# CVMethods/gabor_color_image_segmentation

Hardware: AMD Instinct MI355X
Metric: Mpix/s segmented (Gabor+k-means), 481x321x3 batch (higher is better)
Workload: dtype i8; 1 GPU; batch 64/GPU synthetic 481x321x3 uint8 (seed 0), 4-scale x 6-orientation Gabor bank ksize 13 on a 2-level octave pyramid, k=8, n_iter=10; codebook=global, global_batch=64, parallelism=dp1 (images sharded, int64 centroid all-reduce)

## Files before the change

### gabor_color_image_segmentation_amd/csrc/lloyd_mfma.hip

```cpp
#include "lloyd_pass.h"


#ifndef GCS_KP_WAVES
#define GCS_KP_WAVES 3
#endif
#ifndef GCS_ABL
#define GCS_ABL 0
#endif
#ifdef GCS_KP_PHASES
__device__ unsigned long long g_kp_phases[1024 * 4 * 8];
extern "C" int gcs_debug_kp_phases(unsigned long long *out) {
    return (int)hipMemcpyFromSymbol(out, HIP_SYMBOL(g_kp_phases), sizeof(unsigned long long) * 1024 * 4 * 8);
}
#define KP_PHASE_DECL unsigned long long kp_ph[6] = {0, 0, 0, 0, 0, 0}, kp_t0 = __builtin_amdgcn_s_memtime(), kp_tiles = 0
#define KP_PHASE(k)                                                   \
    do {                                                              \
        const unsigned long long t_ = __builtin_amdgcn_s_memtime();   \
        kp_ph[k] += t_ - kp_t0;                                       \
        kp_t0 = t_;                                                   \
    } while (0)
#define KP_PHASE_STORE                                                                                           \
    do {                                                                                                         \
        const int wg_ = (int)(blockIdx.y * gridDim.x + blockIdx.x);                                              \
        if (lane == 0 && wg_ < 1024) {                                                                           \
            for (int k_ = 0; k_ < 6; ++k_) g_kp_phases[(wg_ * 4 + (wid & 3)) * 8 + k_] = kp_ph[k_];             \
            g_kp_phases[(wg_ * 4 + (wid & 3)) * 8 + 6] = kp_tiles;                                               \
        }                                                                                                        \
    } while (0)
#else
#define KP_PHASE_DECL
#define KP_PHASE(k)
#define KP_PHASE_STORE
#endif

template <int KT, int NST, int DSTEPS, int WAVES, bool SPLIT = false, int L0T = 0, bool FUSED = false>
__global__ __launch_bounds__(64 * WAVES, (WAVES == 8 ? 2
                                          : DSTEPS == KP_DSTEPS_NARROW && KT == 1 && NST <= (SPLIT ? 3 : 6) ? GCS_KP_WAVES
                                          : DSTEPS == KP_DSTEPS_NARROW ? 2 : 1)) void kmeans_pass_mfma_kernel(
    const unsigned char *__restrict__ feats, const uint16_t *__restrict__ cent, GcsLayout lo, int K, int per_image,
    int parts, int reverse, int row_lo, int row_hi, uint64_t *__restrict__ partials, void *__restrict__ raster,
    int raster_u8, int nt_flag, GcsFold fz) {
    constexpr int KP_ROWS = 16 * DSTEPS, KP_DSTEPS = DSTEPS, KP_NT = 2 * DSTEPS;
    constexpr int NTHR = 64 * WAVES;
    constexpr int NT_OWN = WAVES == 8 ? (KP_NT + 1) / 2 : KP_NT;
    constexpr int KP_COARSE = DSTEPS == KP_DSTEPS_NARROW ? 40 * 32 + 64 : 104 * 32 + 64;
    __shared__ __attribute__((aligned(16))) unsigned char s_tile[KP_ROWS * KP_PITCH];
    __shared__ __attribute__((aligned(16))) unsigned char s_coarse[KP_COARSE];
    __shared__ __attribute__((aligned(16))) unsigned char s_lab[KP_TP];
    __shared__ long long s_const[16];
    constexpr int KP_FLAGS = 320;
    __shared__ unsigned char s_flag[SPLIT ? KP_FLAGS : 4];
    static_assert(!SPLIT || (DSTEPS == KP_DSTEPS_NARROW && WAVES == 4), "the split slab is the narrow pass's");
    static_assert(!FUSED || (SPLIT && KT == 1), "the self-updating pass exists for the CL1 kernels");

    const bool do_acc = partials != nullptr;
    const int tid = threadIdx.x, lane = tid & 63;
    const int wid = tid >> 6;
    const int wave = wid & 3;
    const int half = wid >> 2;
    const int b = blockIdx.y, part = blockIdx.x;
    const int D = lo.D;
    const uint16_t *cset = cent + (size_t)(per_image ? b : 0) * K * D;
    const int ntiles = lo.ntiles;
    const int nimg = per_image ? 1 : (int)gridDim.y;
    const int G = parts * nimg, g = per_image ? part : b * parts + part;
    const int nlist = ntiles * nimg;
    const unsigned char *fb = feats + (size_t)(per_image ? b : 0) * lo.img_bytes;

    uint16_t *cs = reinterpret_cast<uint16_t *>(s_tile);
    if constexpr (FUSED) {
        const int D1 = D + 1, row_len = K * D1;
        const int set = per_image ? b : 0;
        const int wg = b * (int)gridDim.x + part, nwg = (int)(gridDim.x * gridDim.y);
        {
            const long long total = (long long)(per_image ? (int)gridDim.y : 1) * fz.rows * row_len;
            for (long long i = (long long)wg * NTHR + tid; i < total; i += (long long)nwg * NTHR) fz.clear[i] = 0ull;
        }
        unsigned long long *fsum = reinterpret_cast<unsigned long long *>(s_tile + 8 * KT * KP_ROWS * 2);
        static_assert(8 * KT * KP_ROWS * 2 % 16 == 0 && 8 * KT * KP_ROWS * 2 + 8 * (8 * KT * KP_ROWS) <= KP_ROWS * KP_PITCH,
                      "the folded sums do not fit behind the centroid scratch");
        const bool later = fz.prev != nullptr;
        if (later) {
            const unsigned long long *pv = fz.prev + (size_t)set * fz.rows * row_len;
            for (int i = tid; i < row_len; i += NTHR) {
                unsigned long long s = 0;
                for (int r = 0; r < fz.rows; ++r) s += pv[(size_t)r * row_len + i];
                fsum[i] = s;
            }
            __syncthreads();
        }
        const bool writer = part == 0 && (per_image || b == 0);
        const long long P = (long long)lo.H * lo.W;
        for (int i = tid; i < 8 * KT * KP_ROWS; i += NTHR) {
            const int j = i / KP_ROWS, r = i % KP_ROWS;
            int e = 0;
            if (r >= lo.row0[0] && r < lo.row0[0] + lo.DL[0]) e = kp_logical_of<0>(lo, r - lo.row0[0]);
            if (lo.n_levels > 1 && r >= lo.row0[1] && r < lo.row0[1] + lo.DL[1]) e = kp_logical_of<1>(lo, r - lo.row0[1]);
            unsigned v = 0;
            if (j < K && r < D) {
                if (later) {
                    const unsigned long long c = fsum[j * D1 + D], s = fsum[j * D1 + e];
                    v = c > 0 ? (unsigned)((2 * s + c) / (2 * c)) : (unsigned)cset[j * D + e];
                } else {
                    const long long p = ((2LL * j + 1) * P) / (2LL * K);
                    v = gcs_slab_value(feats, lo, set, r, (int)(p / lo.W), (int)(p % lo.W));
                }
                if (writer) {
                    fz.cent_new[((size_t)set * K + j) * D + e] = (uint16_t)v;
                    fz.cent_out[((size_t)set * K + j) * D + e] = (uint16_t)v;
                }
                v ^= 0x8080u;
            }
            cs[i] = (uint16_t)v;
        }
    } else
    for (int i = tid; i < 8 * KT * KP_ROWS; i += NTHR) {
        const int j = i / KP_ROWS, r = i % KP_ROWS;
        int e = 0;
        if (r >= lo.row0[0] && r < lo.row0[0] + lo.DL[0]) e = kp_logical_of<0>(lo, r - lo.row0[0]);
        if (lo.n_levels > 1 && r >= lo.row0[1] && r < lo.row0[1] + lo.DL[1]) e = kp_logical_of<1>(lo, r - lo.row0[1]);
        if (lo.n_levels > 2 && r >= lo.row0[2] && r < lo.row0[2] + lo.DL[2]) e = kp_logical_of<2>(lo, r - lo.row0[2]);
        if (lo.n_levels > 3 && r >= lo.row0[3] && r < lo.row0[3] + lo.DL[3]) e = kp_logical_of<3>(lo, r - lo.row0[3]);
        cs[i] = (j < K && r < D) ? (uint16_t)(cset[j * D + e] ^ 0x8080u) : (uint16_t)0;
    }
    if constexpr (SPLIT) {
        for (int it = tid; it < KP_FLAGS; it += NTHR) {
            const long long lt = (long long)g + (long long)it * G;
            unsigned char f = 0;
            if (lt < nlist) {
                const int T = reverse ? nlist - 1 - (int)lt : (int)lt;
                const int bi = T / ntiles, tn = T - bi * ntiles;
                f = *reinterpret_cast<const unsigned *>(fb + (size_t)bi * lo.img_bytes + lo.flag_off + 4 * (size_t)tn) != 0u;
            }
            s_flag[it] = f;
        }
    }
    __syncthreads();
    {
      for (int j = tid >> 4; j < 16; j += NTHR / 16) {
        const int sub = tid & 15;
        long long nrm = 0, scl = 0, sch = 0;
        if (j < K)
            for (int d = sub; d < D; d += 16) {
                const long long c = cs[j * KP_ROWS + d] ^ 0x8080u;
                nrm += c * c;
                scl += c & 255;
                sch += c >> 8;
            }
#pragma unroll
        for (int m = 8; m >= 1; m >>= 1) {
            nrm += __shfl_xor(nrm, m);
            scl += __shfl_xor(scl, m);
            sch += __shfl_xor(sch, m);
        }
        if (sub == 0) {
            const long long q = 16384LL * D;
            const long long g = (128 * scl - q) + 256 * (128 * (sch + scl) - 2 * q) + 65536 * (128 * sch - q);
            s_const[j] = j < K ? 16 * (nrm - 2 * g) + j : (1LL << 62) + j;
        }
      }
    }
    v4i apat[KT][KP_DSTEPS];
    {
        const int r = lane & 31, h = lane >> 5;
        const int jj = r >> 2, pat = r & 3;
        const unsigned msk = pat == 0 ? 0x00ff00ffu : pat == 1 ? 0xffffffffu : pat == 2 ? 0xff00ff00u : 0u;
        const unsigned sel = pat == 1 ? 0x02030001u : 0x03020100u;
#pragma unroll
        for (int mt = 0; mt < KT; ++mt)
#pragma unroll
            for (int kk = 0; kk < KP_DSTEPS; ++kk) {
                const v4i w = *reinterpret_cast<const v4i *>(&cs[(8 * mt + jj) * KP_ROWS + 16 * kk + 8 * h]);
                v4i f;
#pragma unroll
                for (int e = 0; e < 4; ++e) f[e] = (int)(__builtin_amdgcn_perm(0u, (unsigned)w[e], sel) & msk);
                apat[mt][kk] = f;
            }
    }
    __syncthreads();
    constexpr bool CL1 = SPLIT && KT == 1;
    const int DL0 = lo.DL[0];
    auto row_addr = [&](int r) -> int {
        return CL1 && r >= DL0 ? DL0 * KP_PITCH + (r - DL0) * KP_P1 : r * KP_PITCH;
    };
    auto row_swz = [&](int r) -> int { return CL1 && r < DL0 ? ((r >> 3) & 1) * 32 : 0; };
    if (tid < (CL1 ? 32 : KP_TP / 2)) reinterpret_cast<unsigned *>(&s_tile[row_addr(D)])[tid] = 0x01010101u;
    constexpr bool UPD2 = SPLIT && KT == 1;
    constexpr int NACC = UPD2 ? DSTEPS : NT_OWN;
    v4i accu[NACC];
#pragma unroll
    for (int nt = 0; nt < NACC; ++nt) accu[nt] = v4i{0, 0, 0, 0};

    const int n0 = SPLIT ? 16 * lo.DL[0] : 32 * lo.DL[0];
    const int n1 = lo.n_levels > 1 ? 8 * lo.DL[1] : 0;
    const int nchunk = SPLIT ? lo.S >> 4 : lo.tile_bytes >> 4;
    v4i st[NST];
    v2i sm[NST], stt[NST];
#pragma unroll
    for (int i = 0; i < NST; ++i) stt[i] = v2i{0, 0};
    int sdst[NST], ssrc[NST];
    int scls[NST];
    bool sl1[NST];
#pragma unroll
    for (int i = 0; i < NST; ++i) {
        const int ci = min(tid + NTHR * i, nchunk - 1);
        ssrc[i] = ci;
        const int c1 = ci - n0;
        const bool l1 = SPLIT ? c1 >= 0 : c1 >= 0 && c1 < n1;
        sl1[i] = l1;
        if constexpr (SPLIT)
            sdst[i] = l1 ? (CL1 ? (int)(size_t)&s_tile[row_addr(lo.row0[1] + (c1 >> 2)) + (c1 & 3) * 32]
                                : (int)(size_t)&s_tile[(lo.row0[1] + (c1 >> 2)) * KP_PITCH + (c1 & 3) * 32])
                         : (int)(size_t)&s_tile[(ci >> 4) * KP_PITCH + (((ci & 1) * 256 + ((ci & 15) >> 1) * 16) ^ row_swz(ci >> 4))];
        else
            sdst[i] = ci < n0 ? (int)(size_t)&s_tile[(ci >> 5) * KP_PITCH + (ci & 31) * 16]
                      : l1    ? (int)(size_t)&s_tile[(lo.row0[1] + (c1 >> 3)) * KP_PITCH + (c1 & 7) * 64]
                              : (int)(size_t)&s_coarse[(c1 - n1) * 16];
        const unsigned long long m = __builtin_amdgcn_ballot_w64(l1);
        scls[i] = m == 0ull ? 0 : m == ~0ull ? 1 : 2;
    }
    auto stage_load = [&](int tile) {
        const v4i *src = reinterpret_cast<const v4i *>(fb + (size_t)tile * lo.tile_bytes);
#pragma unroll
        for (int i = 0; i < NST; ++i) st[i] = src[ssrc[i]];
    };
    auto stage_load_split = [&](const unsigned char *p_lo, unsigned mid_rel, bool top, bool nt) {
        const __amdgpu_buffer_rsrc_t rs = __builtin_amdgcn_make_buffer_rsrc(const_cast<unsigned char *>(p_lo), 0, -1, 0x00020000);
        const unsigned top_rel = mid_rel + (unsigned)(lo.top_off - lo.mid_off);
        auto go = [&](auto aux_c) {
            constexpr int AUX = decltype(aux_c)::value;
#pragma unroll
            for (int i = 0; i < NST; ++i) {
                const unsigned o = (unsigned)ssrc[i] * 16u;
                st[i] = __builtin_bit_cast(v4i, __builtin_amdgcn_raw_buffer_load_b128(rs, (int)o, 0, AUX));
                sm[i] = __builtin_bit_cast(v2i, __builtin_amdgcn_raw_buffer_load_b64(rs, (int)(o >> 1), (int)mid_rel, AUX));
            }
            if (top) {
#pragma unroll
                for (int i = 0; i < NST; ++i)
                    stt[i] = __builtin_bit_cast(v2i, __builtin_amdgcn_raw_buffer_load_b64(rs, (int)((unsigned)ssrc[i] * 8u), (int)top_rel, AUX));
            } else {
#pragma unroll
                for (int i = 0; i < NST; ++i) {
                    v2i u;
                    asm("" : "=v"(u));
                    stt[i] = u;
                }
            }
        };
        if (nt) go(std::integral_constant<int, 2>{});
        else go(std::integral_constant<int, 0>{});
    };
    typedef __attribute__((address_space(3))) v4i *lds_v4i_ptr;
    bool top_regs = false;
    auto stage_write_as = [&](auto topp) {
    constexpr bool TOPP = decltype(topp)::value;
    auto split_hi = [&](unsigned mid, unsigned top, unsigned &e, unsigned &o) {
        if constexpr (TOPP) {
            e = ((mid & 0x0f0f0f0fu) | ((top << 4) & 0xf0f0f0f0u)) ^ 0x80808080u;
            o = (((mid >> 4) & 0x0f0f0f0fu) | (top & 0xf0f0f0f0u)) ^ 0x80808080u;
        } else {
            e = (mid & 0x0f0f0f0fu) | 0x80808080u;
            o = ((mid >> 4) & 0x0f0f0f0fu) | 0x80808080u;
        }
    };
    {
#pragma unroll
        for (int i = 0; i < NST; ++i) {
            const v4i v = st[i];
            if constexpr (SPLIT) {
                const v2i m = sm[i], t = stt[i];
                auto level0 = [&]() {
#pragma unroll
                    for (int g = 0; g < 2; ++g) {
                        unsigned e, o;
                        split_hi((unsigned)m[g], (unsigned)t[g], e, o);
                        const unsigned a = (unsigned)v[2 * g], bb = (unsigned)v[2 * g + 1];
                        v4i w;
                        if constexpr (CL1) {
                            w[0] = (int)__builtin_amdgcn_perm(e, a, 0x06020400u);
                            w[1] = (int)__builtin_amdgcn_perm(o, bb, 0x06020400u);
                            w[2] = (int)__builtin_amdgcn_perm(e, a, 0x07030501u);
                            w[3] = (int)__builtin_amdgcn_perm(o, bb, 0x07030501u);
                        } else {
                            w[0] = (int)__builtin_amdgcn_perm(e, a, 0x05010400u);
                            w[1] = (int)__builtin_amdgcn_perm(e, a, 0x07030602u);
                            w[2] = (int)__builtin_amdgcn_perm(o, bb, 0x05010400u);
                            w[3] = (int)__builtin_amdgcn_perm(o, bb, 0x07030602u);
                        }
                        *reinterpret_cast<lds_v4i_ptr>(sdst[i] + 128 * g) = w;
                    }
                };
                auto level1 = [&]() {
                    const int e16 = ((lane >> 2) & 1) * 16;
                    if constexpr (CL1) {
#pragma unroll
                        for (int j = 0; j < 2; ++j) {
                            unsigned e, o;
                            split_hi((unsigned)m[j], (unsigned)t[j], e, o);
                            const unsigned a0 = (unsigned)v[2 * j], a1 = (unsigned)v[2 * j + 1];
                            v4i w;
                            w[0] = (int)__builtin_amdgcn_perm(e, a0, 0x05010400u);
                            w[1] = (int)__builtin_amdgcn_perm(o, a0, 0x05030402u);
                            w[2] = (int)__builtin_amdgcn_perm(e, a1, 0x07010600u);
                            w[3] = (int)__builtin_amdgcn_perm(o, a1, 0x07030602u);
                            *reinterpret_cast<lds_v4i_ptr>(sdst[i] + 16 * j) = w;
                        }
                        return;
                    }
#pragma unroll
                    for (int j = 0; j < 2; ++j) {
                        unsigned e, o;
                        split_hi((unsigned)m[j], (unsigned)t[j], e, o);
#pragma unroll
                        for (int qq = 0; qq < 2; ++qq) {
                            const unsigned a = (unsigned)v[2 * j + qq];
                            const unsigned w0 = __builtin_amdgcn_perm(e, a, qq ? 0x07010600u : 0x05010400u);
                            const unsigned w1 = __builtin_amdgcn_perm(o, a, qq ? 0x07030602u : 0x05030402u);
                            v4i w;
                            w[0] = (int)__builtin_amdgcn_perm(0u, w0, 0x01000100u);
                            w[1] = (int)__builtin_amdgcn_perm(0u, w0, 0x03020302u);
                            w[2] = (int)__builtin_amdgcn_perm(0u, w1, 0x01000100u);
                            w[3] = (int)__builtin_amdgcn_perm(0u, w1, 0x03020302u);
                            const int d = sdst[i] + 128 * (2 * j + qq);
                            *reinterpret_cast<lds_v4i_ptr>(d + e16) = w;
                            *reinterpret_cast<lds_v4i_ptr>(d + 16 - e16) = w;
                        }
                    }
                };
                if (GCS_ABL & 4) {
                    *reinterpret_cast<lds_v4i_ptr>(sdst[i]) = v;
                    *reinterpret_cast<lds_v4i_ptr>(sdst[i] + 128) = v4i{m[0], m[1], t[0], t[1]};
                } else
                if (scls[i] == 0) level0();
                else if (scls[i] == 1) level1();
                else if (sl1[i]) level1();
                else level0();
            } else if (scls[i] == 0) {
                *reinterpret_cast<lds_v4i_ptr>(sdst[i]) = v;
            } else {
                const bool f = (lane >> 2) & 1;
                const unsigned x0 = f ? (unsigned)v[2] : (unsigned)v[0], x1 = f ? (unsigned)v[3] : (unsigned)v[1];
                const unsigned y0 = f ? (unsigned)v[0] : (unsigned)v[2], y1 = f ? (unsigned)v[1] : (unsigned)v[3];
                v4i ra, rb;
                ra[0] = (int)__builtin_amdgcn_perm(0u, x0, 0x01000100u);
                ra[1] = (int)__builtin_amdgcn_perm(0u, x0, 0x03020302u);
                ra[2] = (int)__builtin_amdgcn_perm(0u, x1, 0x01000100u);
                ra[3] = (int)__builtin_amdgcn_perm(0u, x1, 0x03020302u);
                rb[0] = (int)__builtin_amdgcn_perm(0u, y0, 0x01000100u);
                rb[1] = (int)__builtin_amdgcn_perm(0u, y0, 0x03020302u);
                rb[2] = (int)__builtin_amdgcn_perm(0u, y1, 0x01000100u);
                rb[3] = (int)__builtin_amdgcn_perm(0u, y1, 0x03020302u);
                if (scls[i] == 1 || sl1[i]) {
                    const int e16 = ((lane >> 1) & 1) * 16, f32 = f ? 32 : 0;
                    *reinterpret_cast<lds_v4i_ptr>(sdst[i] + f32 + e16) = ra;
                    *reinterpret_cast<lds_v4i_ptr>(sdst[i] + f32 + 16 - e16) = ra;
                    *reinterpret_cast<lds_v4i_ptr>(sdst[i] + 32 - f32 + e16) = rb;
                    *reinterpret_cast<lds_v4i_ptr>(sdst[i] + 32 - f32 + 16 - e16) = rb;
                } else {
                    *reinterpret_cast<lds_v4i_ptr>(sdst[i]) = v;
                }
            }
        }
    }
    };
    auto stage_write = [&]() {
        if (SPLIT && top_regs) stage_write_as(std::true_type{});
        else stage_write_as(std::false_type{});
    };
    auto expand_deep = [&]() {
        for (int L = 2; L < lo.n_levels; ++L) {
            const int side = 8 >> L;
            const unsigned char *srcL = s_coarse + (lo.off[L] - lo.off[2]);
            const int items = lo.DL[L] * 32;
            for (int it = tid; it < items; it += NTHR) {
                const int rr = it >> 5, grp = it & 31;
                const int blkq = grp >> 3, iy = grp & 7;
                const unsigned char *s = srcL + (((rr * 4 + blkq) * side + (iy >> L)) * side) * 2;
                v4i o;
                if (L == 2) {
                    const unsigned v = *reinterpret_cast<const unsigned *>(s);
                    o[0] = o[1] = (int)__builtin_amdgcn_perm(0u, v, 0x01000100u);
                    o[2] = o[3] = (int)__builtin_amdgcn_perm(0u, v, 0x03020302u);
                } else {
                    const unsigned v = *reinterpret_cast<const uint16_t *>(s);
                    o[0] = o[1] = o[2] = o[3] = (int)(v | (v << 16));
                }
                *reinterpret_cast<v4i *>(&s_tile[(lo.row0[L] + rr) * KP_PITCH + (blkq * 64 + iy * 8) * 2]) = o;
            }
        }
    };

    const int un = lane & 15, ug = lane >> 4;
    unsigned a_tr[KP_DSTEPS][2], a_up[KP_DSTEPS][2];
    if constexpr (CL1) {
        const int i16 = lane & 15, pxblk = (lane >> 4) & 1, hh = lane >> 5;
#pragma unroll
        for (int kk = 0; kk < KP_DSTEPS; ++kk)
#pragma unroll
            for (int rd = 0; rd < 2; ++rd) {
                const int r = 16 * kk + 8 * hh + (i16 >> 2) + 4 * rd;
                const int off = r < DL0 ? ((wave * 64 + 16 * pxblk + 4 * (i16 & 3)) * 2) ^ row_swz(r) : pxblk * 32 + wave * 8;
                a_tr[kk][rd] = (unsigned)(size_t)(__attribute__((address_space(3))) unsigned char *)&s_tile[row_addr(r) + off];
            }
#pragma unroll
        for (int pt = 0; pt < KP_DSTEPS; ++pt) {
            const int r = 16 * pt + un;
            const bool full = r < DL0;
            const int off = full ? ((wave * 64 + 8 * ug) * 2) ^ row_swz(r) : (ug >> 1) * 32 + wave * 8;
            a_up[pt][0] = (unsigned)(size_t)(__attribute__((address_space(3))) unsigned char *)&s_tile[row_addr(r) + off];
            a_up[pt][1] = a_up[pt][0] + (full ? 8u : 0u);
        }
    }
    const unsigned usel = (un & 1) ? 0x07050301u : 0x06040200u;
    const unsigned eqr = (unsigned)un * 0x01010101u;
    const int cnt_bp = 2 * D;

    auto phys = [&](int lt) { return reverse ? nlist - 1 - lt : lt; };
    int ltile = g;
    if constexpr (!SPLIT) {
        if (ltile < nlist) stage_load(phys(ltile));
    }
    const int s1 = __builtin_amdgcn_readfirstlane(G % ntiles);
    const int q1 = __builtin_amdgcn_readfirstlane(4 * s1 / lo.bx_n), r1 = 4 * s1 - q1 * lo.bx_n;
    const int q2 = __builtin_amdgcn_readfirstlane(4 * (ntiles - s1) / lo.bx_n), r2 = 4 * (ntiles - s1) - q2 * lo.bx_n;
    int tin = __builtin_amdgcn_readfirstlane(phys(g < nlist ? g : 0) % ntiles);
    int by, bx;
    {
        const int blk0 = 4 * tin + wave;
        by = blk0 / lo.bx_n;
        bx = blk0 - by * lo.bx_n;
    }
    if constexpr (SPLIT) {
        by = __builtin_amdgcn_readfirstlane(by);
        bx = __builtin_amdgcn_readfirstlane(bx);
    }
    const int qG = __builtin_amdgcn_readfirstlane(G / ntiles);
    int tin_l = tin, it_l = 0;
    const unsigned char *p_lo_l = nullptr;
    unsigned mid_rel_l = 0;
    long long d_lo[2] = {0, 0};
    int d_rel[2] = {0, 0};
    if constexpr (SPLIT) {
        const int bi0 = __builtin_amdgcn_readfirstlane(phys(g < nlist ? g : 0) / ntiles);
        const unsigned char *img = fb + (size_t)bi0 * lo.img_bytes;
        p_lo_l = img + (size_t)tin * lo.S;
        mid_rel_l = (unsigned)(lo.mid_off - (size_t)tin * (lo.S >> 1));
        const long long sg = reverse ? -1 : 1;
        d_lo[0] = sg * ((long long)qG * lo.img_bytes + (long long)s1 * lo.S);
        d_lo[1] = sg * ((long long)(qG + 1) * lo.img_bytes + (long long)(s1 - ntiles) * lo.S);
        d_rel[0] = (int)(sg * -(long long)s1 * (lo.S >> 1));
        d_rel[1] = (int)(sg * -(long long)(s1 - ntiles) * (lo.S >> 1));
    }
    auto tile_has_top = [&](int it) -> bool {
        return __builtin_amdgcn_readfirstlane(it < KP_FLAGS ? (int)s_flag[it < KP_FLAGS ? it : 0] : 1) != 0;
    };
    const int nt_limit = __builtin_amdgcn_readfirstlane(nt_flag);
    auto load_next_split = [&](bool top, int pos) {
        top_regs = top;
        stage_load_split(p_lo_l, mid_rel_l, top_regs, pos < nt_limit);
        const int tn = reverse ? tin_l - s1 : tin_l + s1;
        const bool wrap = reverse ? tn < 0 : tn >= ntiles;
        tin_l = wrap ? (reverse ? tn + ntiles : tn - ntiles) : tn;
        p_lo_l += wrap ? d_lo[1] : d_lo[0];
        mid_rel_l += (unsigned)(wrap ? d_rel[1] : d_rel[0]);
        ++it_l;
    };
    if constexpr (SPLIT) {
        if (ltile < nlist) load_next_split(tile_has_top(0), ltile);
    }
    long long kbase[KT][4];
    if constexpr (CL1) {
#pragma unroll
        for (int mt = 0; mt < KT; ++mt)
#pragma unroll
            for (int g4 = 0; g4 < 4; ++g4) kbase[mt][g4] = s_const[8 * mt + 2 * g4 + (lane >> 5)];
    }
    KP_PHASE_DECL;
    for (; ltile < nlist; ltile += G) {
        const int tile = phys(ltile);
        int flag_next = 1;
        if constexpr (SPLIT) flag_next = it_l < KP_FLAGS ? (int)s_flag[it_l < KP_FLAGS ? it_l : 0] : 1;
        stage_write();
        KP_PHASE(0);
        __syncthreads();
        KP_PHASE(1);
        __builtin_amdgcn_s_setprio(3);
        if (ltile + G < nlist) {
            if constexpr (SPLIT) load_next_split(__builtin_amdgcn_readfirstlane(flag_next) != 0, ltile + G);
            else stage_load(phys(ltile + G));
        }
        __builtin_amdgcn_s_setprio(0);
        KP_PHASE(2);
        if (!SPLIT && lo.n_levels > 2) {
            expand_deep();
            __syncthreads();
        }

        const int blk = 4 * tin + wave;
        const bool full_blk = CL1 && !raster && blk < lo.nmain && 8 * bx + 8 <= lo.W && 8 * by >= row_lo &&
                              8 * by + 8 <= (row_hi < lo.H ? row_hi : lo.H);
#pragma unroll
        for (int sub_i = 0; sub_i < ((GCS_ABL & 1) ? 0 : WAVES == 8 ? 1 : 2); ++sub_i) {
            const int sub = WAVES == 8 ? half : sub_i;
            const int n = lane & 31, h = lane >> 5;
            const int pl = wave * 64 + sub * 32 + n;
            v16i acc[KT];
#pragma unroll
            for (int mt = 0; mt < KT; ++mt)
#pragma unroll
                for (int e = 0; e < 16; ++e) acc[mt][e] = 0;
            v4i bfr[KP_DSTEPS];
            {
                const int i16 = lane & 15, pxblk = (lane >> 4) & 1;
                const unsigned addr = (unsigned)(size_t)&s_tile[(8 * h + (i16 >> 2)) * KP_PITCH +
                                                                (wave * 64 + sub * 32 + 16 * pxblk + 4 * (i16 & 3)) * 2];
                v2i fa[KP_DSTEPS], fbv[KP_DSTEPS];
                if constexpr (CL1) {
#pragma unroll
                    for (int kk = 0; kk < KP_DSTEPS; ++kk)
                        asm volatile("ds_read_b64_tr_b16 %0, %2 offset:%c4\n\t"
                                     "ds_read_b64_tr_b16 %1, %3 offset:%c4"
                                     : "=&v"(fa[kk]), "=&v"(fbv[kk])
                                     : "v"(a_tr[kk][0]), "v"(a_tr[kk][1]), "i"(sub * 64)
                                     : "memory");
                } else
#pragma unroll
                for (int kk = 0; kk < KP_DSTEPS; ++kk)
                    asm volatile("ds_read_b64_tr_b16 %0, %2\n\t"
                                 "ds_read_b64_tr_b16 %1, %2 offset:%c3"
                                 : "=&v"(fa[kk]), "=&v"(fbv[kk])
                                 : "v"(addr + kk * 16 * KP_PITCH), "i"(4 * KP_PITCH)
                                 : "memory");
                asm volatile("s_waitcnt lgkmcnt(0)" ::: "memory");
#pragma unroll
                for (int kk = 0; kk < KP_DSTEPS; ++kk) {
                    asm volatile("" : "+v"(fa[kk]), "+v"(fbv[kk]));
                    bfr[kk] = v4i{fa[kk][0], fa[kk][1], fbv[kk][0], fbv[kk][1]};
                }
            }
#pragma unroll
            for (int kk = 0; kk < KP_DSTEPS; ++kk)
#pragma unroll
                for (int mt = 0; mt < KT; ++mt)
                    acc[mt] = __builtin_amdgcn_mfma_i32_32x32x32_i8(apat[mt][kk], bfr[kk], acc[mt], 0, 0, 0);
            long long best = 0x7fffffffffffffffLL;
#pragma unroll
            for (int mt = 0; mt < KT; ++mt)
#pragma unroll
                for (int g = 0; g < 4; ++g) {
                    const int u = __mul24(acc[mt][4 * g + 1], 256) + acc[mt][4 * g];
                    long long key = mad_i64_i32(u, -32, CL1 ? kbase[mt][g] : s_const[8 * mt + 2 * g + h]);
                    key = mad_i64_i32(acc[mt][4 * g + 2], -2097152, key);
                    best = key < best ? key : best;
                }
            const unsigned blo = (unsigned)best, bhi = (unsigned)((unsigned long long)best >> 32);
            const auto s0 = __builtin_amdgcn_permlane32_swap(blo, blo, false, false);
            const auto s1 = __builtin_amdgcn_permlane32_swap(bhi, bhi, false, false);
            const long long ka = (long long)(((unsigned long long)s1[0] << 32) | s0[0]);
            const long long kb = (long long)(((unsigned long long)s1[1] << 32) | s0[1]);
            const int bj = (int)((kb < ka ? s0[1] : s0[0]) & 15);
            if (h == 0 && CL1 && full_blk) {
                s_lab[pl] = (unsigned char)bj;
            } else
            if (h == 0) {
                const auto col_of = [&](int nn) { return CL1 ? 2 * (nn & 3) + ((nn >> 2) & 1) : nn & 7; };
                int y = 8 * by + 4 * sub + (n >> 3), x = 8 * bx + col_of(n), xlim = lo.W;
                if (blk >= lo.nmain) {
                    int no = n;
                    asm volatile("" : "+v"(no));
                    gcs_strip_pixel(lo, blk, 4 * sub + (no >> 3), col_of(no), y, x, xlim);
                }
                const bool inimg = blk < lo.nblk && y < lo.H && x < xlim;
                const bool valid = inimg && y >= row_lo && y < row_hi;
                s_lab[pl] = valid ? (unsigned char)bj : (unsigned char)0xFF;
                if (raster && inimg) {
                    const size_t o = ((size_t)(per_image ? b : tile / ntiles) * lo.H + y) * lo.W + x;
                    if (raster_u8) static_cast<uint8_t *>(raster)[o] = (uint8_t)bj;
                    else static_cast<int32_t *>(raster)[o] = bj;
                }
            }
        }
        KP_PHASE(3);
        if (WAVES == 8 && do_acc) __syncthreads();
        if constexpr (UPD2) {
          if (do_acc && !(GCS_ABL & 2)) {
            const unsigned eqj = (unsigned)(un >> 1) * 0x01010101u;
            const unsigned sel01 = (un & 1) ? 0x010c000cu : 0x0c010c00u, sel23 = (un & 1) ? 0x030c020cu : 0x0c030c02u;
#pragma unroll
            for (int hf = 0; hf < 2; ++hf) {
                const v2i lw = *reinterpret_cast<const v2i *>(&s_lab[wave * 64 + hf * 32 + 8 * ug]);
                v4i oh;
#pragma unroll
                for (int i = 0; i < 2; ++i) {
                    const unsigned x = (unsigned)lw[i] ^ eqj;
                    const unsigned y = (x | 0x80808080u) - 0x01010101u;
                    const unsigned d = ~y & 0x80808080u;
                    oh[2 * i] = (int)__builtin_amdgcn_perm(0u, d, sel01);
                    oh[2 * i + 1] = (int)__builtin_amdgcn_perm(0u, d, sel23);
                }
                static_assert(DSTEPS == 5, "the update's read batch is written out for five plane tiles");
                v4i bq[DSTEPS];
                v2i bl[DSTEPS], bh[DSTEPS];
#pragma unroll
                for (int pt = 0; pt < DSTEPS; ++pt) {
                    if (pt < L0T)
                        asm volatile("ds_read_b128 %0, %1 offset:%c2" : "=&v"(bq[pt]) : "v"(a_up[pt][0]), "i"(hf * 64) : "memory");
                    else
                        asm volatile("ds_read_b64 %0, %2 offset:%c4\n\t"
                                     "ds_read_b64 %1, %3 offset:%c4"
                                     : "=&v"(bl[pt]), "=&v"(bh[pt])
                                     : "v"(a_up[pt][0]), "v"(a_up[pt][1]), "i"(hf * 64)
                                     : "memory");
                }
#define KP_UPD_YOUNGER(pt_) (((pt_) + 1 < L0T ? L0T - 1 - (pt_) : 0) + 2 * (DSTEPS - ((pt_) + 1 < L0T ? L0T : (pt_) + 1)))
#define KP_UPD_STEP(pt_)                                                                                  \
    do {                                                                                                  \
        asm volatile("s_waitcnt lgkmcnt(%0)" ::"n"(KP_UPD_YOUNGER(pt_)) : "memory");                       \
        if ((pt_) < L0T) {                                                                                \
            asm volatile("" : "+v"(bq[pt_]));                                                             \
        } else {                                                                                          \
            asm volatile("" : "+v"(bl[pt_]), "+v"(bh[pt_]));                                              \
            bq[pt_] = v4i{bl[pt_][0], bl[pt_][1], bh[pt_][0], bh[pt_][1]};                                \
        }                                                                                                 \
        accu[pt_] = __builtin_amdgcn_mfma_i32_16x16x64_i8(oh, bq[pt_], accu[pt_], 0, 0, 0);               \
    } while (0)
                KP_UPD_STEP(0);
                KP_UPD_STEP(1);
                KP_UPD_STEP(2);
                KP_UPD_STEP(3);
                KP_UPD_STEP(4);
#undef KP_UPD_STEP
#undef KP_UPD_YOUNGER
            }
          }
        } else
        if (do_acc && !(GCS_ABL & 2)) {
            const v4i lw = *reinterpret_cast<const v4i *>(&s_lab[wave * 64 + 16 * ug]);
            v4i oh;
#pragma unroll
            for (int i = 0; i < 4; ++i) {
                const unsigned x = (unsigned)lw[i] ^ eqr;
                const unsigned y = (x | 0x80808080u) - 0x01010101u;
                oh[i] = (int)(~y & 0x80808080u);
            }
#pragma unroll
            for (int nti = 0; nti < NT_OWN; ++nti) {
                const int nt = WAVES == 8 ? min(half * NT_OWN + nti, KP_NT - 1) : nti;
                const int d = 8 * nt + (un >> 1);
                const v4i *src = reinterpret_cast<const v4i *>(&s_tile[d * KP_PITCH + (wave * 64 + 16 * ug) * 2]);
                const v4i w0 = src[0], w1 = src[1];
                v4i bx_;
                bx_[0] = (int)__builtin_amdgcn_perm((unsigned)w0[1], (unsigned)w0[0], usel);
                bx_[1] = (int)__builtin_amdgcn_perm((unsigned)w0[3], (unsigned)w0[2], usel);
                bx_[2] = (int)__builtin_amdgcn_perm((unsigned)w1[1], (unsigned)w1[0], usel);
                bx_[3] = (int)__builtin_amdgcn_perm((unsigned)w1[3], (unsigned)w1[2], usel);
                accu[nti] = __builtin_amdgcn_mfma_i32_16x16x64_i8(oh, bx_, accu[nti], 0, 0, 0);
            }
        }
        {
            const int tn = reverse ? tin - s1 : tin + s1;
            const bool wrap = reverse ? tn < 0 : tn >= ntiles;
            const bool up = reverse == wrap;
            const int dq = wrap ? q2 : q1, dr = wrap ? r2 : r1;
            tin = wrap ? (reverse ? tn + ntiles : tn - ntiles) : tn;
            if (up) {
                bx += dr;
                by += dq;
                if (bx >= lo.bx_n) { bx -= lo.bx_n; ++by; }
            } else {
                bx -= dr;
                by -= dq;
                if (bx < 0) { bx += lo.bx_n; --by; }
            }
        }
        KP_PHASE(4);
        __syncthreads();
        KP_PHASE(5);
#ifdef GCS_KP_PHASES
        ++kp_tiles;
#endif
    }
    KP_PHASE_STORE;

    if constexpr (FUSED) {
        if (!do_acc && fz.prev != nullptr) {
            __shared__ int s_last;
            const int nwg = (int)(gridDim.x * gridDim.y);
            if (tid == 0) s_last = atomicAdd(fz.ticket, 1u) == (unsigned)(nwg - 1);
            __syncthreads();
            if (s_last) {
                const long long total = (long long)(per_image ? (int)gridDim.y : 1) * fz.rows * K * (D + 1);
                for (long long i = tid; i < total; i += NTHR) fz.prev[i] = 0ull;
                if (tid == 0) *fz.ticket = 0u;
            }
        }
    }
    if (!do_acc) return;
    if constexpr (UPD2) {
        constexpr int RW2 = 16 * DSTEPS;
        int *red = reinterpret_cast<int *>(s_tile);
        static_assert(4 * 16 * RW2 * 4 <= KP_ROWS * KP_PITCH, "fold buffer exceeds the tile buffer");
#pragma unroll
        for (int pt = 0; pt < DSTEPS; ++pt)
#pragma unroll
            for (int e = 0; e < 4; ++e) red[(wave * 16 + 4 * ug + e) * RW2 + 16 * pt + un] = accu[pt][e];
        __syncthreads();
        const int D1 = D + 1;
        auto folded = [&](int j, int bb, int plane) {
            int sm_ = 0;
#pragma unroll
            for (int w = 0; w < 4; ++w) sm_ += red[(w * 16 + 2 * j + bb) * RW2 + plane];
            return -(long long)sm_ / 128;
        };
        for (int i = tid; i < K * D1; i += NTHR) {
            const int j = i / D1, e = i % D1;
            const long long nj = folded(j, 0, D);
            long long out = nj;
            if (e < D) {
                const int c = e / lo.F, f = e - c * lo.F;
                int pe = kp_plane_on_level<0>(lo, c, f);
                { const int q = kp_plane_on_level<1>(lo, c, f); pe = q >= 0 ? q : pe; }
                { const int q = kp_plane_on_level<2>(lo, c, f); pe = q >= 0 ? q : pe; }
                { const int q = kp_plane_on_level<3>(lo, c, f); pe = q >= 0 ? q : pe; }
                out = (folded(j, 0, pe) + 128 * nj) + 256 * (folded(j, 1, pe) + 128 * nj);
            }
            if constexpr (FUSED) {
                const int wg = b * (int)gridDim.x + part;
                unsigned long long *row = reinterpret_cast<unsigned long long *>(partials) +
                                          ((size_t)(per_image ? b : 0) * fz.rows + (size_t)(wg % fz.rows)) * (K * D1);
                if (out != 0) atomicAdd(&row[i], (unsigned long long)out);
            } else
            partials[partial_index(per_image, b, part, parts, (int)gridDim.y, i, K * D1)] = (uint64_t)out;
        }
    }
    if constexpr (!UPD2) {
    constexpr int RW = KP_NT * 16;
    int *red = reinterpret_cast<int *>(s_tile);
    static_assert(4 * 16 * RW * 4 <= KP_ROWS * KP_PITCH, "fold buffer exceeds the tile buffer");
#pragma unroll
    for (int nti = 0; nti < NT_OWN; ++nti) {
        const int nt = WAVES == 8 ? half * NT_OWN + nti : nti;
        if (nt < KP_NT)
#pragma unroll
            for (int e = 0; e < 4; ++e) red[(wave * 16 + 4 * ug + e) * RW + 16 * nt + un] = accu[nti][e];
    }
    __syncthreads();
    const int D1 = D + 1;
    auto folded = [&](int j, int bp) {
        int s = 0;
#pragma unroll
        for (int w = 0; w < 4; ++w) s += red[(w * 16 + j) * RW + bp];
        return -(long long)s / 128;
    };
    for (int i = tid; i < K * D1; i += NTHR) {
        const int j = i / D1, e = i % D1;
        const long long nj = folded(j, cnt_bp);
        long long out = nj;
        if (e < D) {
            const int c = e / lo.F, f = e - c * lo.F;
            int pe = kp_plane_on_level<0>(lo, c, f);
            { const int q = kp_plane_on_level<1>(lo, c, f); pe = q >= 0 ? q : pe; }
            { const int q = kp_plane_on_level<2>(lo, c, f); pe = q >= 0 ? q : pe; }
            { const int q = kp_plane_on_level<3>(lo, c, f); pe = q >= 0 ? q : pe; }
            out = (folded(j, 2 * pe) + 128 * nj) + 256 * (folded(j, 2 * pe + 1) + 128 * nj);
        }
        partials[partial_index(per_image, b, part, parts, (int)gridDim.y, i, K * D1)] = (uint64_t)out;
    }
    }
}

template <int KT, int NST, int DSTEPS, int WAVES, bool SPLIT, int L0T, bool FUSED>
static void launch_mfma_as(const LloydPassArgs &a, const GcsFold &fz, int nt_flag) {
    hipLaunchKernelGGL((kmeans_pass_mfma_kernel<KT, NST, DSTEPS, WAVES, SPLIT, L0T, FUSED>), dim3(a.parts, a.B), dim3(64 * WAVES), 0,
                       a.stream, a.feats, a.cent, a.lo, a.k, a.n_sets == a.B ? 1 : 0, a.parts, a.reverse ? 1 : 0, a.row_lo, a.row_hi,
                       a.partials, a.lab_out, a.lab_u8, nt_flag, fz);
}
template <bool SELF, int KT, int NST, int DSTEPS, int WAVES, bool SPLIT, int L0T>
static void launch_mfma(const LloydPassArgs &a, const GcsFold *fz, int nt_flag) {
    if constexpr (SELF)
        if (fz) return launch_mfma_as<KT, NST, DSTEPS, WAVES, SPLIT, L0T, true>(a, *fz, nt_flag);
    launch_mfma_as<KT, NST, DSTEPS, WAVES, SPLIT, L0T, false>(a, GcsFold{}, nt_flag);
}

void lloyd_mfma_launch(GcsPassKernel pk, const LloydPassArgs &a, const GcsFold *fz) {
    const int nt_flag = gcs_pass_nt_limit(pk, a.lo, a.B, a.n_sets);
    switch (pk) {
#define GCS_PASS_LAUNCH(id, name, ...)                                                      \
    case GCS_PASS_##id:                                                                     \
        return launch_mfma<gcs_pass_self_updating(GCS_PASS_##id), __VA_ARGS__>(a, fz, nt_flag);
        GCS_MFMA_PASSES(GCS_PASS_LAUNCH)
#undef GCS_PASS_LAUNCH
    default: return;
    }
}
```

Baseline: 5670 Mpix/s.

## Add label-only pass variant that defers raster stores to the next tile iteration

Adds a MAP_ONLY template form of the k-means MFMA pass, selected when labels are requested without partial accumulation. Instead of writing each pixel's label directly to global memory inside the compute loop, labels go to shared memory and are flushed after the next tile's barrier, so the global stores overlap the next stage load and compute. Accumulation code is compiled out for this form. The cost is extra per-tile bookkeeping (image, block coordinates) and one more kernel instantiation per pass type, which adds code size and register pressure.

```diff
diff --git a/gabor_color_image_segmentation_amd/csrc/lloyd_mfma.hip b/gabor_color_image_segmentation_amd/csrc/lloyd_mfma.hip
--- a/gabor_color_image_segmentation_amd/csrc/lloyd_mfma.hip
+++ b/gabor_color_image_segmentation_amd/csrc/lloyd_mfma.hip
@@ -33,7 +33,7 @@
 #define KP_PHASE_STORE
 #endif
 
-template <int KT, int NST, int DSTEPS, int WAVES, bool SPLIT = false, int L0T = 0, bool FUSED = false>
+template <int KT, int NST, int DSTEPS, int WAVES, bool SPLIT = false, int L0T = 0, bool FUSED = false, bool MAP_ONLY = false>
 __global__ __launch_bounds__(64 * WAVES, (WAVES == 8 ? 2
                                           : DSTEPS == KP_DSTEPS_NARROW && KT == 1 && NST <= (SPLIT ? 3 : 6) ? GCS_KP_WAVES
                                           : DSTEPS == KP_DSTEPS_NARROW ? 2 : 1)) void kmeans_pass_mfma_kernel(
@@ -53,7 +53,7 @@
     static_assert(!SPLIT || (DSTEPS == KP_DSTEPS_NARROW && WAVES == 4), "the split slab is the narrow pass's");
     static_assert(!FUSED || (SPLIT && KT == 1), "the self-updating pass exists for the CL1 kernels");
 
-    const bool do_acc = partials != nullptr;
+    const bool do_acc = !MAP_ONLY && partials != nullptr;
     const int tid = threadIdx.x, lane = tid & 63;
     const int wid = tid >> 6;
     const int wave = wid & 3;
@@ -476,15 +476,52 @@
 #pragma unroll
             for (int g4 = 0; g4 < 4; ++g4) kbase[mt][g4] = s_const[8 * mt + 2 * g4 + (lane >> 5)];
     }
+    constexpr bool defer = MAP_ONLY;
+    int img = __builtin_amdgcn_readfirstlane(phys(g < nlist ? g : 0) / ntiles);
+    bool pend = false;
+    int p_tin = 0, p_by = 0, p_bx = 0, p_img = 0, lab_prev = 0;
+    auto lab_slot = [&]() {
+        int l_ = lane;
+        asm volatile("" : "+v"(l_));
+        const int r = WAVES == 8 ? 4 * half + ((l_ >> 3) & 3) : l_ >> 3, c = l_ & 7;
+        return wave * 64 + 8 * r + (CL1 ? (c >> 1) + 4 * (c & 1) : c);
+    };
+    auto store_labels = [&](int lab) {
+        const int blk = 4 * p_tin + wave;
+        if (blk >= lo.nblk) return;
+        int l_ = lane;
+        asm volatile("" : "+v"(l_));
+        const int r = WAVES == 8 ? 4 * half + ((l_ >> 3) & 3) : l_ >> 3, c = l_ & 7;
+        const bool act = WAVES == 8 ? l_ < 32 : true;
+        const size_t row0 = (size_t)(per_image ? b : p_img) * lo.H;
+        if (blk < lo.nmain && 8 * p_bx + 8 <= lo.W && 8 * p_by + 8 <= lo.H) {
+            const size_t base = (row0 + 8 * p_by) * lo.W + 8 * p_bx;
+            const int off = r * lo.W + c;
+            if (act) {
+                if (raster_u8) (static_cast<uint8_t *>(raster) + base)[off] = (uint8_t)lab;
+                else (static_cast<int32_t *>(raster) + base)[off] = lab;
+            }
+        } else {
+            int y = 8 * p_by + r, x = 8 * p_bx + c, xlim = lo.W;
+            if (blk >= lo.nmain) gcs_strip_pixel(lo, blk, r, c, y, x, xlim);
+            if (act && y < lo.H && x < xlim) {
+                const size_t o = (row0 + y) * lo.W + x;
+                if (raster_u8) static_cast<uint8_t *>(raster)[o] = (uint8_t)lab;
+                else static_cast<int32_t *>(raster)[o] = lab;
+            }
+        }
+    };
     KP_PHASE_DECL;
     for (; ltile < nlist; ltile += G) {
         const int tile = phys(ltile);
         int flag_next = 1;
         if constexpr (SPLIT) flag_next = it_l < KP_FLAGS ? (int)s_flag[it_l < KP_FLAGS ? it_l : 0] : 1;
+        if (CL1 && defer && pend) lab_prev = s_lab[lab_slot()];
         stage_write();
         KP_PHASE(0);
         __syncthreads();
         KP_PHASE(1);
+        if (defer && pend) store_labels(CL1 ? lab_prev : (int)s_lab[lab_slot()]);
         __builtin_amdgcn_s_setprio(3);
         if (ltile + G < nlist) {
             if constexpr (SPLIT) load_next_split(__builtin_amdgcn_readfirstlane(flag_next) != 0, ltile + G);
@@ -560,7 +597,7 @@
             const long long ka = (long long)(((unsigned long long)s1[0] << 32) | s0[0]);
             const long long kb = (long long)(((unsigned long long)s1[1] << 32) | s0[1]);
             const int bj = (int)((kb < ka ? s0[1] : s0[0]) & 15);
-            if (h == 0 && CL1 && full_blk) {
+            if (h == 0 && (defer || (CL1 && full_blk))) {
                 s_lab[pl] = (unsigned char)bj;
             } else
             if (h == 0) {
@@ -658,9 +695,17 @@
                 accu[nti] = __builtin_amdgcn_mfma_i32_16x16x64_i8(oh, bx_, accu[nti], 0, 0, 0);
             }
         }
+        if constexpr (MAP_ONLY) {
+            p_tin = tin;
+            p_by = __builtin_amdgcn_readfirstlane(by);
+            p_bx = __builtin_amdgcn_readfirstlane(bx);
+            p_img = img;
+            pend = true;
+        }
         {
             const int tn = reverse ? tin - s1 : tin + s1;
             const bool wrap = reverse ? tn < 0 : tn >= ntiles;
+            if constexpr (MAP_ONLY) img += reverse ? -(qG + (int)wrap) : qG + (int)wrap;
             const bool up = reverse == wrap;
             const int dq = wrap ? q2 : q1, dr = wrap ? r2 : r1;
             tin = wrap ? (reverse ? tn + ntiles : tn - ntiles) : tn;
@@ -682,6 +727,7 @@
 #endif
     }
     KP_PHASE_STORE;
+    if (defer && pend) store_labels(s_lab[lab_slot()]);
 
     if constexpr (FUSED) {
         if (!do_acc && fz.prev != nullptr) {
@@ -770,11 +816,16 @@
     }
 }
 
+template <int KT, int NST, int DSTEPS, int WAVES, bool SPLIT, int L0T, bool FUSED, bool MAP_ONLY>
+static void launch_mfma_form(const LloydPassArgs &a, const GcsFold &fz, int nt_flag) {
+    hipLaunchKernelGGL((kmeans_pass_mfma_kernel<KT, NST, DSTEPS, WAVES, SPLIT, L0T, FUSED, MAP_ONLY>), dim3(a.parts, a.B),
+                       dim3(64 * WAVES), 0, a.stream, a.feats, a.cent, a.lo, a.k, a.n_sets == a.B ? 1 : 0, a.parts, a.reverse ? 1 : 0,
+                       a.row_lo, a.row_hi, a.partials, a.lab_out, a.lab_u8, nt_flag, fz);
+}
 template <int KT, int NST, int DSTEPS, int WAVES, bool SPLIT, int L0T, bool FUSED>
 static void launch_mfma_as(const LloydPassArgs &a, const GcsFold &fz, int nt_flag) {
-    hipLaunchKernelGGL((kmeans_pass_mfma_kernel<KT, NST, DSTEPS, WAVES, SPLIT, L0T, FUSED>), dim3(a.parts, a.B), dim3(64 * WAVES), 0,
-                       a.stream, a.feats, a.cent, a.lo, a.k, a.n_sets == a.B ? 1 : 0, a.parts, a.reverse ? 1 : 0, a.row_lo, a.row_hi,
-                       a.partials, a.lab_out, a.lab_u8, nt_flag, fz);
+    if (a.lab_out && !a.partials) launch_mfma_form<KT, NST, DSTEPS, WAVES, SPLIT, L0T, FUSED, true>(a, fz, nt_flag);
+    else launch_mfma_form<KT, NST, DSTEPS, WAVES, SPLIT, L0T, FUSED, false>(a, fz, nt_flag);
 }
 template <bool SELF, int KT, int NST, int DSTEPS, int WAVES, bool SPLIT, int L0T>
 static void launch_mfma(const LloydPassArgs &a, const GcsFold *fz, int nt_flag) {
```

New measurement: 5670 Mpix/s (median of 5 runs). No clear change (-0.0%).
